# LZ-QWQ/Multi-modal-Tracking

Measured on AMD Instinct MI355X. Metric: tracker FPS (template+search fwd) MixViT-B RGB-T @320px, 1/2/4/8 MI355X, higher is better.
Workload: dtype bf16; 1 GPU; mixformer_vit_rgbt (two-stream) ViT-B 128px template x2 + 320px search, RGB+TIR, 1 frame(s)/GPU/step; variant=rgbt, batch_per_gpu=1, template=128, search=320, hidden=768, depth=12, parallelism=single, hip_graph=True

## Files before the change

multi-modal-tracking_amd/csrc/gemm_glds.hip:

```cpp
#include "common.hpp"
#include "gemm_internal.hpp"

#include <algorithm>

#ifndef MMT_GEMM_ABLATE
#define MMT_GEMM_ABLATE 0
#endif
#ifndef MMT_GEMM_GM
#define MMT_GEMM_GM 8
#endif
#ifndef MMT_GEMM_AB
#define MMT_GEMM_AB 0
#endif
#ifndef MMT_GEMM_OCC2_RES
#define MMT_GEMM_OCC2_RES 1
#endif
#ifndef MMT_GEMM_SK_TICKET_FIRST
#define MMT_GEMM_SK_TICKET_FIRST 0
#endif
#ifndef MMT_GEMM_SK8_MIN
#define MMT_GEMM_SK8_MIN 64
#endif
#ifndef MMT_GEMM_NO_OCC2
#define MMT_GEMM_NO_OCC2 0
#endif

#if MMT_STAMP_BUILD
__device__ unsigned long long g_mmt_stamps[16384 * 8];
extern "C" int mmt_gemm_stamps(unsigned long long* host, int n) {
    return (int)hipMemcpyFromSymbol(host, HIP_SYMBOL(g_mmt_stamps), sizeof(unsigned long long) * n);
}
#endif
#define MMT_STAMP(I, INSN) MMT_STAMP_AT(g_mmt_stamps, I, INSN)

namespace {

template <int N>
struct gemm_ic {
    static constexpr int value = N;
};

typedef __attribute__((address_space(3))) void lds_void;
typedef __attribute__((address_space(1))) void glb_void;

template <int N>
MMT_DEV void wait_vm() {
    asm volatile("s_waitcnt vmcnt(%0)" ::"n"(N) : "memory");
}

MMT_DEV void glds16(const void* src, unsigned char* dst) {
    __builtin_amdgcn_global_load_lds((glb_void*)src, (lds_void*)dst, 16, 0, 0);
}

template <int L, int ST>
MMT_DEV void wait_stages(int ahead) {
    static_assert(ST <= 4, "wait table written for ST <= 4");
    if (ahead <= 0) wait_vm<0>();
    else if (ahead == 1) wait_vm<L>();
    else if (ahead == 2 || ST < 4) wait_vm<(ST >= 3 ? 2 * L : L)>();
    else wait_vm<(ST >= 4 ? 3 * L : L)>();
}

__device__ __attribute__((aligned(64))) const uint32_t g_zero_chunk[16] = {0};
__device__ __attribute__((aligned(64))) const uint32_t g_one_chunk_bf16[4] = {0x3F80u, 0u, 0u, 0u};
__device__ __attribute__((aligned(64))) const uint32_t g_one_chunk_f16[4] = {0x3C00u, 0u, 0u, 0u};

template <int OFF>
MMT_DEV uint2 gemm_tr16(const unsigned char* p) {
    uint2 r;
    const uint32_t a = (uint32_t)(uintptr_t)(const __attribute__((address_space(3))) unsigned char*)p;
    asm volatile("ds_read_b64_tr_b16 %0, %1 offset:%2" : "=v"(r) : "v"(a), "n"(OFF));
    return r;
}

MMT_DEV int gemm_trsw(int k) { return 2 * ((k & 3) | (((k >> 3) & 1) << 2)); }

struct gemm_lean_null {
    MMT_DEV constexpr decltype(nullptr) operator[](int) const { return nullptr; }
};
struct gemm_lean_fixed {
    static constexpr int64_t a_seg_rows = INT32_MAX, a_segs_a = 1, a_stride_a = 0, a_stride_b = 0;
    static constexpr int64_t c_seg_rows = 0, c_seg_pitch = 0;
    static constexpr int32_t k_split = 0, conv_h = 0, conv_up = 1, conv_cin = 0, conv_k3 = 0;
    static constexpr int32_t r_mode = 0, r_p0 = 1, r_p1 = 1, r_t = 0;
    static constexpr float* sk_ws = nullptr;
    static constexpr uint32_t* sk_cnt = nullptr;
    static constexpr int64_t sk_cnt_n = 0;
    gemm_lean_null a1;
};
struct gemm_lean_grid {
    int32_t per_g;
    int32_t tn_magic;
    int32_t q8, r8;
    float inv_k;
};
template <int EPI, int ACT>
struct gemm_lean_args;
template <int ACT>
struct gemm_lean_args<1, ACT> : gemm_lean_fixed, gemm_lean_grid {
    const void *a[2], *w[2];
    const float *bias[2], *ln_colsum[2], *ln_stats_in[2];
    void* c[2];
    int32_t M, N, K, lda, ldc;
    float ln_eps;
    static constexpr int32_t act = ACT, c2_copy = 0, ldr = 0;
    gemm_lean_null r, c2, ln_stats_out;
};
template <int ACT>
struct gemm_lean_args<2, ACT> : gemm_lean_fixed, gemm_lean_grid {
    const void *a[2], *w[2];
    const float *bias[2], *r[2];
    void *c[2], *c2[2];
    float* ln_stats_out[2];
    int32_t M, N, K, lda, ldc, ldr;
    static constexpr int32_t act = 0, c2_copy = 1;
    static constexpr float ln_eps = 0.f;
    gemm_lean_null ln_colsum, ln_stats_in;
};
template <typename P>
struct gemm_is_lean { static constexpr bool value = false; };
template <int EPI, int ACT>
struct gemm_is_lean<gemm_lean_args<EPI, ACT>> { static constexpr bool value = true; };

template <typename T, int BM, int BN, int WGM, int WGN, int KS, int ST, bool CONV, int LNM, int OCC = 1, bool RS = false,
          int EPI = 0, typename P = mmt_gemm_params>
MMT_DEV void gemm_glds_tile(const P& p, const int g, const int tile, const int slice, const int nsk,
                            const int ntiles) {
    constexpr int NW = WGM * WGN, TPG = 64 * NW;
    constexpr int KT = 64;
    constexpr int STAGE = (BM + BN) * 128;
    constexpr int PA = BM / 8 / NW, PB = BN / 8 / NW;
    static_assert(PA * 8 * NW == BM && PB * 8 * NW == BN, "pieces divide evenly over the waves");
    constexpr int L = PA + PB;
    constexpr int WM = BM / WGM, WN = BN / WGN, MT = WM / 16, NT = WN / 16;
    static_assert(KS * ST * STAGE <= 160 * 1024, "LDS budget");
    constexpr bool SB = BM * BN >= 256 * 256 || OCC > 1;
    constexpr bool W4 = BM == 256 && BN == 256 && NW == 4;
    static_assert(!W4 || (KS == 1 && ST == 2 && OCC == 1 && !CONV && (LNM == 0 || LNM == 2)), "impl 9 geometry");
    static_assert(!SB || (KS == 1 && (LNM == 0 || LNM >= 2) && !CONV), "impl 7 / 8 / 9: plain GEMM (or handed-in LN statistics)");
    constexpr bool TA = LNM == 4, TB = LNM == 3 || LNM == 4;
    static_assert(!TB || (BM == 128 && BN == 128 && !CONV), "MN-major operands: 128x128 tiles");
    static_assert(KS == 1 || BM * BN * 4 <= KS * ST * STAGE, "k-group reduction buffer");
    constexpr bool LEAN = gemm_is_lean<P>::value;
    static_assert(!LEAN || (OCC == 1 && !CONV && !RS && (LNM == 0 || LNM == 2) && BM * BN <= 128 * 128 &&
                            ((EPI == 1 && LNM == 2) || (EPI == 2 && LNM == 0))), "lean frame kernels");
    constexpr int LDS_BYTES = W4 ? (BM / 2) * (BN + 4) * 4 + BM * 8 + 64 : KS * ST * STAGE;
    static_assert(LDS_BYTES >= KS * ST * STAGE && LDS_BYTES <= 160 * 1024, "LDS budget");
    __shared__ __attribute__((aligned(1024))) unsigned char lds[LDS_BYTES];
    MMT_STAMP(0, "s_memrealtime");
    MMT_STAMP(1, "s_memtime");

    const int tiles_m = (p.M + BM - 1) / BM;
    constexpr int GM = MMT_GEMM_GM;
    int tm, tn;
    if ((BM * BN >= 256 * 128 || OCC > 1) && gridDim.x * gridDim.y * gridDim.z > 512 && tiles_m > GM) {
        const int tiles_n = ntiles / tiles_m, grp = tile / (GM * tiles_n), first = grp * GM;
        const int gsz = min(tiles_m - first, GM), r = tile - grp * GM * tiles_n;
        tm = first + r % gsz;
        tn = r / gsz;
    } else if constexpr (LEAN) {
        tn = (int)(((uint32_t)tile * (uint32_t)p.tn_magic) >> 16);
        tm = tile - tn * tiles_m;
    } else {
        tm = tile % tiles_m;
        tn = tile / tiles_m;
    }
    constexpr bool LNF = LNM == 1 || LNM == 2;
    const int m0_tile = tm * BM, n0 = tn * BN;
    const int lane = threadIdx.x & 63, kg = threadIdx.x / TPG;
    const int wid = (threadIdx.x % TPG) >> 6, wr = wid / WGN, wc = wid % WGN;
    const int l16 = lane & 15, lg = lane >> 4;
    const int M = p.M, N = p.N, K = p.K;

    const T* A0 = (const T*)p.a[g];
    const T* A1 = (const T*)p.a1[g];
    const T* W = (const T*)p.w[g];

    const int prow = lane >> 3, pch = (lane & 7) ^ prow;
    int64_t aoff[PA], boff[PB];
    int ay[PA], ax[PA];
    const int ch = p.conv_h, cup = CONV ? p.conv_up : 1, hi = CONV ? p.conv_h / cup : 0;
    if constexpr (!CONV) {
        const int segr = (int)p.a_seg_rows, sega = (int)p.a_segs_a;
        const bool plain = segr >= M;
#pragma unroll
        for (int i = 0; i < PA; ++i) {
            const int m = min(m0_tile + (wid * PA + i) * 8 + prow, M - 1);
            if (plain) {
                aoff[i] = (int64_t)m * p.lda;
            } else {
                const int seg = m / segr, sa = seg % sega;
                aoff[i] = sa * p.a_stride_a + (int64_t)((seg - sa) / sega) * p.a_stride_b + (int64_t)(m - seg * segr) * p.lda;
            }
            ay[i] = ax[i] = 0;
        }
    } else {
#pragma unroll
        for (int i = 0; i < PA; ++i) {
            const int m = min(m0_tile + (wid * PA + i) * 8 + prow, M - 1);
            const int b = m / (ch * ch), rem = m - b * ch * ch;
            ay[i] = rem / ch;
// ... 316 lines not shown
#pragma unroll
                for (int nt = 0; nt < NT; ++nt)
#pragma unroll
                    for (int mt = 0; mt < MT; ++mt) acc[nt][mt] += __builtin_bit_cast(f32x4, v[nt][mt]);
            }
        }
    }

    constexpr int TP = BN + 4;
    constexpr int EPASS = BM * TP * 4 + KS * BM * 8 + 16 <= KS * ST * STAGE ? 1 : WGM, EB = BM / EPASS;
    static_assert(EPASS == 1 || (EB == WM && KS == 1 && (LNM == 0 || LNM >= 2)),
                  "multi-pass epilogue: plain GEMM tiles (also with handed-in LayerNorm statistics)");
    static_assert(EB * TP * 4 + KS * BM * 8 + 4 <= LDS_BYTES, "epilogue pass fits in LDS");
    constexpr int FLAG_OFF = EB * TP * 4 + KS * BM * 8;
    float* ctile = (float*)lds;
    float* rstat = ctile + EB * TP;
    constexpr int NTH_E = TPG * KS, TPRW = NTH_E / BM;
    static_assert(TPRW >= 1 && (TPRW & (TPRW - 1)) == 0 && TPRW <= 64, "statistics reduction geometry");
    constexpr int NSP = TPRW >= 2 ? 8 : 16;
    f32x2 stp[NSP];
    const int kp = K / 64, srow = threadIdx.x / TPRW, spart = threadIdx.x % TPRW;
    if constexpr (LNM == 2) {
        const f32x2* st = (const f32x2*)p.ln_stats_in[g] + (int64_t)min(m0_tile + srow, M - 1) * kp;
#pragma unroll
        for (int i = 0; i < NSP; ++i) {
            const int j = spart + i * TPRW;
            stp[i] = j < kp ? st[j] : f32x2{0.f, 0.f};
        }
    }
    constexpr int TPR0 = BN / 8, RPP0 = TPG * KS / TPR0, NPASS0 = EB / RPP0;
    constexpr bool RPRE = EPASS == 1 && NPASS0 <= 8 && BM * BN <= 128 * 128 && OCC == 1;
    const int tc0 = (threadIdx.x % TPR0) * 8, tr0 = threadIdx.x / TPR0, nc0 = min(n0 + tc0, N - 8);
    auto rload = [&](int m, int nc, f32x4& ra, f32x4& rb) {
        const float* R = p.r[g];
        const int64_t csr = p.c_seg_rows > 0 ? p.c_seg_rows : INT64_MAX, csp = p.c_seg_pitch;
        int64_t rr = csr == INT64_MAX ? (int64_t)m : (m / csr) * csp + m % csr;
        if (p.r_mode == 1) rr = m % p.r_p0;
        else if (p.r_mode == 2) {
            const int hw = p.r_p0 * p.r_p0, b = m / hw, rem = m - b * hw;
            const int y = rem / p.r_p0, x = rem - y * p.r_p0, hs = p.r_p0 / p.r_p1;
            rr = (int64_t)b * hs * hs + (int64_t)(y / p.r_p1) * hs + (x / p.r_p1);
        }
        if (p.r_t) {
            const u32x4 u = *(const u32x4*)((const T*)R + rr * p.ldr + nc);
            const f32x2 u0 = unpack2<T>(u[0]), u1 = unpack2<T>(u[1]), u2 = unpack2<T>(u[2]), u3 = unpack2<T>(u[3]);
            ra = f32x4{u0[0], u0[1], u1[0], u1[1]};
            rb = f32x4{u2[0], u2[1], u3[0], u3[1]};
        } else {
            ra = *(const f32x4*)(R + rr * p.ldr + nc);
            rb = *(const f32x4*)(R + rr * p.ldr + nc + 4);
        }
    };
    f32x4 rpa[RPRE ? NPASS0 : 1], rpb[RPRE ? NPASS0 : 1];
    if constexpr (LEAN && EPI == 2) __builtin_assume(p.r[g] != nullptr);
    const bool rpre = RPRE && p.r[g] != nullptr && nsk == 1;
    if constexpr (RPRE) {
        if (rpre) {
#pragma unroll
            for (int i = 0; i < NPASS0; ++i) rload(min(m0_tile + tr0 + i * RPP0, M - 1), nc0, rpa[i], rpb[i]);
        }
    }
    lds_barrier();
    if constexpr (LNM == 2) {
        float sx = 0.f, sxx = 0.f;
#pragma unroll
        for (int i = 0; i < NSP; ++i) {
            sx += stp[i][0];
            sxx += stp[i][1];
        }
#pragma unroll
        for (int o = 1; o < TPRW; o <<= 1) {
            sx += __shfl_xor(sx, o, 64);
            sxx += __shfl_xor(sxx, o, 64);
        }
        if (spart == 0) {
            rstat[srow * 2] = sx;
            rstat[srow * 2 + 1] = sxx;
        }
    }
    if constexpr (LNM == 1) {
#pragma unroll
        for (int j = 0; j < MTW; ++j) {
            const int mt = wc + j * WGN;
            const float sx = lanegroup_sum(lsx[j]), sxx = lanegroup_sum(lsxx[j]);
            if (mt < MT && lg == 0) {
                rstat[(kg * BM + wr * WM + mt * 16 + l16) * 2] = sx;
                rstat[(kg * BM + wr * WM + mt * 16 + l16) * 2 + 1] = sxx;
            }
        }
    }
    if ((KS == 1 || kg == 1) && (EPASS == 1 || wr == 0)) {
#pragma unroll
        for (int nt = 0; nt < NT; ++nt)
#pragma unroll
            for (int mt = 0; mt < MT; ++mt)
                *(f32x4*)(ctile + ((EPASS == 1 ? wr * WM : 0) + mt * 16 + l16) * TP + wc * WN + nt * 16 + lg * 4) =
                    acc[nt][mt];
    }
    if constexpr (KS == 2) {
        lds_barrier();
        if (kg == 0) {
#pragma unroll
            for (int nt = 0; nt < NT; ++nt)
#pragma unroll
                for (int mt = 0; mt < MT; ++mt) {
                    f32x4* t4 = (f32x4*)(ctile + (wr * WM + mt * 16 + l16) * TP + wc * WN + nt * 16 + lg * 4);
                    *t4 = *t4 + acc[nt][mt];
// ... 90 lines not shown
#pragma unroll
        for (int ps = 0; ps < NPASS; ++ps) {
            const int r = tr + ps * RPP, off = slice * SLAB + (r * BN + tc) * 4;
            __builtin_amdgcn_raw_buffer_store_b128(*(const u32x4*)(ctile + r * TP + tc), slabs, off, 0, 16);
            __builtin_amdgcn_raw_buffer_store_b128(*(const u32x4*)(ctile + r * TP + tc + 4), slabs, off + 16, 0, 16);
        }
        asm volatile("s_waitcnt vmcnt(0)" ::: "memory");
        __syncthreads();
        int* flag = (int*)(lds + FLAG_OFF);
        if (threadIdx.x == 0) {
            const uint32_t old = __hip_atomic_fetch_add(p.sk_cnt + tix, 1u, __ATOMIC_RELAXED, __HIP_MEMORY_SCOPE_AGENT);
            const int last = old == (uint32_t)(nsk - 1);
            if (last) __hip_atomic_store(p.sk_cnt + tix, 0u, __ATOMIC_RELAXED, __HIP_MEMORY_SCOPE_AGENT);
            *flag = last;
        }
        __syncthreads();
        if (!*flag) return;
        __builtin_amdgcn_fence(__ATOMIC_ACQUIRE, "wavefront");
#pragma unroll
        for (int ps = 0; ps < NPASS; ++ps) {
            const int r = tr + ps * RPP, off = (r * BN + tc) * 4;
            f32x4 sa = {0.f, 0.f, 0.f, 0.f}, sb = sa;
#pragma unroll
            for (int q0 = 0; q0 < 8; q0 += 4) {
                u32x4 pa[4], pb[4];
#pragma unroll
                for (int j = 0; j < 4; ++j) {
                    const int q = q0 + j;
                    if (q < nsk && q != slice) {
                        pa[j] = __builtin_amdgcn_raw_buffer_load_b128(slabs, q * SLAB + off, 0, 16);
                        pb[j] = __builtin_amdgcn_raw_buffer_load_b128(slabs, q * SLAB + off + 16, 0, 16);
                    }
                }
#pragma unroll
                for (int j = 0; j < 4; ++j) {
                    const int q = q0 + j;
                    if (q < nsk) {
                        if (q == slice) {
                            sa += *(const f32x4*)(ctile + r * TP + tc);
                            sb += *(const f32x4*)(ctile + r * TP + tc + 4);
                        } else {
                            sa += __builtin_bit_cast(f32x4, pa[j]);
                            sb += __builtin_bit_cast(f32x4, pb[j]);
                        }
                    }
                }
            }
            *(f32x4*)(ctile + r * TP + tc) = sa;
            *(f32x4*)(ctile + r * TP + tc + 4) = sb;
        }
    }
#endif
    if constexpr (LEAN) {
        __builtin_assume(bias != nullptr);
        if constexpr (EPI == 2) {
            __builtin_assume(R != nullptr);
            __builtin_assume(C2 != nullptr);
            __builtin_assume(p.ln_stats_out[g] != nullptr);
        }
    }
    const int n = n0 + tc, nc = min(n, N - 8);
    const bool csplit = p.c2_copy == 3 || p.c2_copy == 4;
    float* stats_out = p.c2_copy && !csplit && C2 ? p.ln_stats_out[g] : nullptr;
    const bool colsplit = csplit && n >= N - 8;
    char* Cs = colsplit ? C2 : C;
    if (csplit) C2 = nullptr;
    f32x4 bn0 = {0.f, 0.f, 0.f, 0.f}, bn1 = bn0, cs0 = bn0, cs1 = bn0;
    if (bias) {
        bn0 = *(const f32x4*)(bias + nc);
        bn1 = *(const f32x4*)(bias + nc + 4);
    }
    if constexpr (LNF) {
        cs0 = *(const f32x4*)(p.ln_colsum[g] + nc);
        cs1 = *(const f32x4*)(p.ln_colsum[g] + nc + 4);
    }
    float inv_k;
    if constexpr (LEAN) inv_k = p.inv_k;
    else inv_k = 1.f / (float)K;
    const int64_t csr = p.c_seg_rows > 0 ? p.c_seg_rows : INT64_MAX, csp = p.c_seg_pitch;
    const uint32_t csr32 = (uint32_t)min(csr, (int64_t)INT32_MAX);
    auto crow = [&](int m) -> int64_t {
        if (csr == INT64_MAX) return (int64_t)m;
        const uint32_t qd = (uint32_t)m / csr32;
        return (int64_t)qd * csp + (int64_t)((uint32_t)m - qd * csr32);
    };
    constexpr int PG = NPASS < 4 ? NPASS : 4;
    for (int ep = 0; ep < EPASS; ++ep) {
    if (ep > 0) {
        lds_barrier();
        if (wr == ep) {
#pragma unroll
            for (int nt = 0; nt < NT; ++nt)
#pragma unroll
                for (int mt = 0; mt < MT; ++mt)
                    *(f32x4*)(ctile + (mt * 16 + l16) * TP + wc * WN + nt * 16 + lg * 4) = acc[nt][mt];
        }
        lds_barrier();
    }
    const int m0 = m0_tile + ep * EB;
    if constexpr (EPI == 1) {
        static_assert(!RS, "compact epilogue: no row scale");
#pragma unroll
        for (int i = 0; i < NPASS; ++i) {
            const int r = tr + i * RPP, m = m0 + r;
            f32x4 va = *(const f32x4*)(ctile + r * TP + tc);
            f32x4 vb = *(const f32x4*)(ctile + r * TP + tc + 4);
            if constexpr (LNF) {
                float sx = 0.f, sxx = 0.f;
                constexpr int NQ = LNM == 1 ? KS : 1;
// ... 171 lines not shown
                    *(f32x4*)((float*)Cs + es + 4) = ob;
                    if (C2 && p.c2_copy == 2) {
                        *(u32x4*)((T*)C2 + e) = u32x4{pack2<T>(prea[0], prea[1]), pack2<T>(prea[2], prea[3]),
                                                      pack2<T>(preb[0], preb[1]), pack2<T>(preb[2], preb[3])};
                    } else if (C2 && p.c2_copy) {
                        *(u32x4*)((T*)C2 + e) = u32x4{pack2<T>(sa[0], sa[1]), pack2<T>(sa[2], sa[3]),
                                                      pack2<T>(sb[0], sb[1]), pack2<T>(sb[2], sb[3])};
                    } else if (C2) {
                        *(f32x4*)((float*)C2 + e) = sa;
                        *(f32x4*)((float*)C2 + e + 4) = sb;
                    }
                } else {
                    *(u32x4*)((T*)Cs + es) = u32x4{pack2<T>(oa[0], oa[1]), pack2<T>(oa[2], oa[3]),
                                                 pack2<T>(ob[0], ob[1]), pack2<T>(ob[2], ob[3])};
                    if (C2 && p.c2_copy == 2)
                        *(u32x4*)((T*)C2 + e) = u32x4{pack2<T>(prea[0], prea[1]), pack2<T>(prea[2], prea[3]),
                                                      pack2<T>(preb[0], preb[1]), pack2<T>(preb[2], preb[3])};
                    else if (C2)
                        *(u32x4*)((T*)C2 + e) = u32x4{pack2<T>(sa[0], sa[1]), pack2<T>(sa[2], sa[3]),
                                                      pack2<T>(sb[0], sb[1]), pack2<T>(sb[2], sb[3])};
                }
            }
        }
    }
    }
    }
    MMT_STAMP(5, "s_memtime");
#if MMT_STAMP_BUILD
    asm volatile("s_waitcnt vmcnt(0)" ::: "memory");
#endif
    MMT_STAMP(6, "s_memtime");
    MMT_STAMP(7, "s_memrealtime");
}

MMT_DEV int gemm_xcd_lin() {
    const int nwg = gridDim.x * gridDim.y * gridDim.z;
    const int orig = blockIdx.x + gridDim.x * (blockIdx.y + gridDim.y * blockIdx.z);
    const int xcd = orig & 7, q8 = nwg >> 3, r8 = nwg & 7;
    return (xcd < r8 ? xcd * (q8 + 1) : r8 * (q8 + 1) + (xcd - r8) * q8) + (orig >> 3);
}

template <typename T, int BM, int BN, int WGM, int WGN, int KS, int ST, bool CONV, int LNM, int EPI = 0>
__global__ __launch_bounds__(64 * WGM * WGN * KS)
    __attribute__((amdgpu_waves_per_eu(WGM * WGN * KS / 4, WGM * WGN * KS / 4))) void gemm_glds_kernel(
        const mmt_gemm_params p) {
    const int nsk = gridDim.y;
    const int lin = gemm_xcd_lin();
    const int per_g = gridDim.x * nsk;
    const int g = lin / per_g, rem_t = lin - g * per_g;
    const int tile = rem_t / nsk, slice = rem_t - tile * nsk;
    gemm_glds_tile<T, BM, BN, WGM, WGN, KS, ST, CONV, LNM, 1, false, EPI>(p, g, tile, slice, nsk, gridDim.x);
}

template <typename T, int BM, int BN, int WGM, int WGN, int KS, int ST, int LNM, int EPI, int ACT>
__global__ __launch_bounds__(64 * WGM * WGN * KS)
    __attribute__((amdgpu_waves_per_eu(WGM * WGN * KS / 4, WGM * WGN * KS / 4))) void gemm_glds_frame_kernel(
        const gemm_lean_args<EPI, ACT> p) {
    const int orig = blockIdx.x, xcd = orig & 7;
    const int lin = xcd * p.q8 + min(xcd, p.r8) + (orig >> 3);
    const int g = lin >= p.per_g ? 1 : 0;
    gemm_glds_tile<T, BM, BN, WGM, WGN, KS, ST, false, LNM, 1, false, EPI>(p, g, lin - g * p.per_g, 0, 1, p.per_g);
}

template <typename T, int BM, int BN, int WGM, int WGN, int KS, int ST, bool RS = false, int EPI = 0, int LNM = 0>
__global__ __launch_bounds__(64 * WGM * WGN * KS)
    __attribute__((amdgpu_waves_per_eu(WGM * WGN * KS / 2, WGM * WGN * KS / 2))) void gemm_glds_kernel_occ2(
        const mmt_gemm_params p) {
    const int nsk = gridDim.y;
    const int lin = gemm_xcd_lin();
    const int per_g = gridDim.x * nsk;
    const int g = lin / per_g, rem_t = lin - g * per_g;
    const int tile = rem_t / nsk, slice = rem_t - tile * nsk;
    gemm_glds_tile<T, BM, BN, WGM, WGN, KS, ST, false, LNM, 2, RS, EPI>(p, g, tile, slice, nsk, gridDim.x);
}

template <typename T, int LNM, int EPI = 0>
__global__ __launch_bounds__(512) __attribute__((amdgpu_waves_per_eu(4, 4))) void gemm_glds_kernel_occ2_t(
    const mmt_gemm_params p) {
    const int nsk = gridDim.y;
    const int lin = gemm_xcd_lin();
    const int per_g = gridDim.x * nsk;
    const int g = lin / per_g, rem_t = lin - g * per_g;
    const int tile = rem_t / nsk, slice = rem_t - tile * nsk;
    gemm_glds_tile<T, 128, 128, 2, 4, 1, 2, false, LNM, 2, false, EPI>(p, g, tile, slice, nsk, gridDim.x);
}

#if MMT_GEMM_AB
template <typename T, int LNM, bool RS = false, int EPI = 0>
__global__ __launch_bounds__(256) __attribute__((amdgpu_waves_per_eu(1, 1))) void gemm_glds_kernel_w4(
    const mmt_gemm_params p) {
    const int lin = gemm_xcd_lin();
    const int g = lin / gridDim.x, tile = lin - g * gridDim.x;
    gemm_glds_tile<T, 256, 256, 2, 2, 1, 2, false, LNM, 1, RS, EPI>(p, g, tile, 0, 1, gridDim.x);
}
#endif

constexpr int GEMM_MULTI = 4;
struct gemm_multi_args {
    mmt_gemm_params p[GEMM_MULTI];
    int32_t wg0[GEMM_MULTI + 1];
    int32_t tiles[GEMM_MULTI];
    int32_t n;
};

template <typename T, int BM, int BN, int WGM, int WGN, int KS, int ST, bool CONV>
__global__ __launch_bounds__(64 * WGM * WGN * KS)
    __attribute__((amdgpu_waves_per_eu(WGM * WGN * KS / 4, WGM * WGN * KS / 4))) void gemm_glds_multi_kernel(
        const gemm_multi_args a) {
    const int lin = gemm_xcd_lin();
    int i = 0;
    while (i + 1 < a.n && lin >= a.wg0[i + 1]) ++i;
    const int loc = lin - a.wg0[i], nt = a.tiles[i];
    const int g = loc / nt;
    gemm_glds_tile<T, BM, BN, WGM, WGN, KS, ST, CONV, 0>(a.p[i], g, loc - g * nt, 0, 1, nt);
// ... 56 lines not shown
        if (residual_epilogue(p, true)) hipLaunchKernelGGL((gemm_glds_kernel_w4<T, 0, true, 2>), grid, block, 0, st, p);
        else hipLaunchKernelGGL((gemm_glds_kernel_w4<T, 0, true>), grid, block, 0, st, p);
    } else if (p.ln_fold == 2) {
        if (compact_epilogue(p)) hipLaunchKernelGGL((gemm_glds_kernel_w4<T, 2, false, 1>), grid, block, 0, st, p);
        else hipLaunchKernelGGL((gemm_glds_kernel_w4<T, 2>), grid, block, 0, st, p);
    } else if (compact_epilogue(p)) {
        hipLaunchKernelGGL((gemm_glds_kernel_w4<T, 0, false, 1>), grid, block, 0, st, p);
    } else if (residual_epilogue(p)) {
        hipLaunchKernelGGL((gemm_glds_kernel_w4<T, 0, false, 2>), grid, block, 0, st, p);
    } else {
        hipLaunchKernelGGL((gemm_glds_kernel_w4<T, 0>), grid, block, 0, st, p);
    }
    return 0;
#endif
}

bool aligned(const void* ptr, int bytes) { return ((uintptr_t)ptr & (uintptr_t)(bytes - 1)) == 0; }

bool glds_takes(const mmt_gemm_params& p) {
    if (p.K % 8 || p.N % 8 || p.ldc % 8 || (p.r[0] && p.ldr % 8)) return false;
    if (p.ln_fold && p.conv_h > 0) return false;
    if (p.ln_fold == 2 && (p.a_seg_rows < p.M || p.k_split || p.K % 64 || p.K > 64 * 8 * 2)) return false;
    for (int g = 0; g < p.groups; ++g) {
        if (p.ln_fold == 2 && (!p.ln_stats_in[g] || !aligned(p.ln_stats_in[g], 8))) return false;
        if (p.ln_stats_out[g] && (!p.c2_copy || !p.c2[g] || p.N % 64 || !aligned(p.ln_stats_out[g], 8))) return false;
    }
    if (p.conv_h > 0) {
        const int cup = p.conv_up, hi = p.conv_up > 0 ? p.conv_h / p.conv_up : 0;
        if (cup <= 0 || (cup & (cup - 1)) || hi * cup != p.conv_h) return false;
        const int64_t imgs = (p.M + (int64_t)p.conv_h * p.conv_h - 1) / ((int64_t)p.conv_h * p.conv_h);
        const int64_t pitch = p.a_stride_a > 0 ? p.a_stride_a : (int64_t)hi * hi;
        if ((imgs * pitch * (int64_t)p.lda + p.K) >= ((int64_t)1 << 32) || p.K >= (1 << 24)) return false;
    }
    if (p.lda % 8 || p.a_stride_a % 8 || p.a_stride_b % 8 || p.k_split % 8) return false;
    if (p.a_seg_rows > INT32_MAX || p.a_segs_a > INT32_MAX) return false;
    for (int g = 0; g < p.groups; ++g) {
        if (!aligned(p.c[g], 16) || (p.c2[g] && !aligned(p.c2[g], 16))) return false;
        if (p.bias[g] && !aligned(p.bias[g], 16)) return false;
        if (p.r[g] && !aligned(p.r[g], 16)) return false;
        if (p.ln_fold && (!p.ln_colsum[g] || !aligned(p.ln_colsum[g], 16))) return false;
    }
    return true;
}

struct Cand { int cfg, bm, bn, ks; float fixed_us, step_us; };
constexpr Cand kCands[7] = {{1, 128, 128, 1, 6.0f, 0.52f}, {2, 128, 64, 2, 5.0f, 0.52f}, {3, 64, 64, 2, 3.2f, 0.33f},
                            {4, 128, 128, 1, 6.0f, 0.60f}, {5, 256, 128, 1, 7.0f, 0.70f}, {6, 128, 256, 1, 7.0f, 0.70f},
                            {7, 256, 256, 1, 9.0f, 1.33f}};
int64_t tiles_of(const mmt_gemm_params& p, int bm, int bn) {
    return (int64_t)((p.M + bm - 1) / bm) * ((p.N + bn - 1) / bn);
}


int lean_cfg(const mmt_gemm_params& p) {
    if (p.groups > 2 || p.K % 64 || p.conv_h > 0 || p.k_split || p.a_seg_rows < p.M || p.c_seg_rows || p.a_t || p.w_t ||
        p.row_scale || p.splitk >= 2 || std::max({p.lda, p.ldc, p.ldr}) > INT32_MAX)
        return 0;
    for (int g = 0; g < p.groups; ++g)
        if (!p.bias[g]) return 0;
    int cfg = 0;
    if (p.ln_fold == 2 && p.c2_copy == 0 && p.act <= 1 && compact_epilogue(p)) {
        cfg = 1;
    } else if (p.ln_fold == 0 && residual_epilogue(p)) {
        for (int g = 0; g < p.groups; ++g)
            if (!p.r[g] || !p.c2[g] || !p.ln_stats_out[g]) return 0;
        cfg = 3;
    } else {
        return 0;
    }
    return tiles_of(p, kCands[cfg - 1].bm, kCands[cfg - 1].bn) * p.groups <= 256 ? cfg : 0;
}

template <typename T, int BM, int BN, int WGM, int WGN, int KS, int ST, int LNM, int EPI, int ACT>
void launch_lean(const mmt_gemm_params& p, hipStream_t st) {
    gemm_lean_args<EPI, ACT> a{};
    const int tiles_m = (p.M + BM - 1) / BM, nwg = (int)tiles_of(p, BM, BN) * p.groups;
    a.per_g = nwg / p.groups;
    a.tn_magic = 65536 / tiles_m + 1;
    a.q8 = nwg >> 3;
    a.r8 = nwg & 7;
    a.inv_k = 1.f / (float)p.K;
    for (int g = 0; g < p.groups; ++g) {
        a.a[g] = p.a[g];
        a.w[g] = p.w[g];
        a.bias[g] = p.bias[g];
        a.c[g] = p.c[g];
        if constexpr (EPI == 1) {
            a.ln_colsum[g] = p.ln_colsum[g];
            a.ln_stats_in[g] = p.ln_stats_in[g];
        } else {
            a.r[g] = p.r[g];
            a.c2[g] = p.c2[g];
            a.ln_stats_out[g] = p.ln_stats_out[g];
        }
    }
    a.M = p.M, a.N = p.N, a.K = p.K, a.lda = (int32_t)p.lda, a.ldc = (int32_t)p.ldc;
    if constexpr (EPI == 1) a.ln_eps = p.ln_eps;
    else a.ldr = (int32_t)p.ldr;
    hipLaunchKernelGGL((gemm_glds_frame_kernel<T, BM, BN, WGM, WGN, KS, ST, LNM, EPI, ACT>), dim3(nwg),
                       dim3(64 * WGM * WGN * KS), 0, st, a);
}

}

template <typename T>
int mmt_gemm_glds(const mmt_gemm_params& p, hipStream_t st, int force) {
    if (force < 0 || !glds_takes(p)) return 1;
    const int lcfg = lean_cfg(p);
    const bool no_lean = force == 10;
    if (force == 10) force = lcfg;
    const int nk = (p.K + 63) / 64;
    const Cand* cands = kCands;
    auto max_split = [&](const Cand& c) -> int {
        if (p.ln_fold || !p.sk_ws || !p.sk_cnt) return 1;
        const int64_t t = tiles_of(p, c.bm, c.bn) * p.groups;
        if (2 * t > p.sk_cnt_n) return 1;
        int n = 8;
        while (n > 1 && ((int64_t)n * c.ks > nk || t * n * c.bm * c.bn > p.sk_ws_floats)) --n;
        return n;
    };
    auto cost = [&](const Cand& c, int n) {
        const int64_t wg = tiles_of(p, c.bm, c.bn) * p.groups * n;
        const int steps = (nk + n - 1) / n;
        const float red = n > 1 ? 0.8f + 0.5f * (float)(n - 1) * (float)(c.bm * c.bn) / 16384.f : 0.f;
        return (float)((wg + 255) / 256) * (c.fixed_us + (float)((steps + c.ks - 1) / c.ks) * c.step_us) + red;
    };
    int cfg = force, nsk = 1;
    if (p.row_scale) {
        if (force == 9) return launch_w4<T>(p, st);
        if ((force != 0 && force != 8) || p.ln_fold || p.conv_h > 0 || p.a_t || p.w_t) return 1;
        const dim3 grid((unsigned)tiles_of(p, 128, 128), 1, p.groups);
        if (residual_epilogue(p, true))
            hipLaunchKernelGGL((gemm_glds_kernel_occ2<T, 128, 128, 2, 4, 1, 2, true, 2>), grid, dim3(512), 0, st, p);
        else
            hipLaunchKernelGGL((gemm_glds_kernel_occ2<T, 128, 128, 2, 4, 1, 2, true>), grid, dim3(512), 0, st, p);
        return 0;
    }
    if (p.a_t || p.w_t) {
        if (force != 0 && force != 1 && force != 8) return 1;
        const int64_t t8 = tiles_of(p, 128, 128) * p.groups;
        const bool big = t8 > 256;
        const Cand& c = cands[0];
        if (force == 0 && p.a_t && t8 >= MMT_GEMM_SK8_MIN && p.splitk == 0 && max_split(c) > 1) {
            cfg = 8;
            nsk = (int)std::min<int64_t>(max_split(c), (480 + t8 - 1) / t8);
        } else if (force == 1 || (force == 0 && !big)) {
            cfg = 1;
            const int nmax = p.splitk >= 1 ? std::min(p.splitk, max_split(c)) : max_split(c);
            float best = 1e30f;
            for (int n = (p.splitk >= 2 ? nmax : 1); n <= nmax; ++n) {
                const float t = cost(c, n) * (n > 1 && p.splitk == 0 ? 1.15f : 1.f);
                if (t < best) best = t, nsk = n;
            }
        } else {
            cfg = 8;
            if (p.splitk >= 2) nsk = std::min(p.splitk, max_split(c));
        }
        const int lnm = p.a_t ? 4 : 3;
        const dim3 grid((unsigned)tiles_of(p, 128, 128), nsk, p.groups);
        if (cfg == 8) {
            if (lnm == 4) hipLaunchKernelGGL((gemm_glds_kernel_occ2_t<T, 4>), grid, dim3(512), 0, st, p);
            else if (compact_epilogue(p)) hipLaunchKernelGGL((gemm_glds_kernel_occ2_t<T, 3, 1>), grid, dim3(512), 0, st, p);
            else hipLaunchKernelGGL((gemm_glds_kernel_occ2_t<T, 3>), grid, dim3(512), 0, st, p);
        } else {
            if (lnm == 4) hipLaunchKernelGGL((gemm_glds_kernel<T, 128, 128, 2, 4, 1, 4, false, 4>), grid, dim3(512), 0, st, p);
            else hipLaunchKernelGGL((gemm_glds_kernel<T, 128, 128, 2, 4, 1, 4, false, 3>), grid, dim3(512), 0, st, p);
        }
        return 0;
    }
    if (cfg == 0) {
        float best = 1e30f;
        const bool big = tiles_of(p, 128, 128) * p.groups > 256;
        const bool big7 = big && !p.ln_fold && p.conv_h == 0 && p.act != 1;
        for (int ci = 0; ci < (big7 ? 7 : big ? 6 : 3); ++ci) {
            if (ci == 3 || ci == 4) continue;
            if (ci == 6) {
                const float t = cost(cands[ci], 1);
                if (t < best) best = t, cfg = 7, nsk = 1;
                continue;
            }
            const Cand& c = cands[ci];
            const int nmax = p.splitk >= 1 ? std::min(p.splitk, max_split(c)) : max_split(c);
            for (int n = (p.splitk >= 2 ? nmax : 1); n <= nmax; ++n) {
                const float t = cost(c, n) * (n > 1 && p.splitk == 0 ? 1.15f : 1.f);
                if (t < best) best = t, cfg = c.cfg, nsk = n;
            }
        }
        if (!MMT_GEMM_NO_OCC2 && big && nsk == 1 && p.ln_fold != 1 && p.conv_h == 0 &&
            (MMT_GEMM_OCC2_RES || !p.ln_stats_out[0]) &&
            (cfg == 1 || cfg == 5 || cfg == 6 || cfg == 7 || (p.ln_fold == 2 && (cfg == 2 || cfg == 3))))
            cfg = 8;
    } else if (cfg == 8) {
        nsk = 1;
    } else if (cfg >= 1 && cfg <= 7) {
        const Cand& c = cands[cfg - 1];
        if (no_lean) {
            nsk = 1;
        } else if (p.splitk >= 2) {
            nsk = std::min(p.splitk, max_split(c));
        } else if (p.splitk == 0) {
            float best = 1e30f;
            for (int n = 1; n <= max_split(c); ++n) {
                const float t = cost(c, n) * (n > 1 ? 1.15f : 1.f);
                if (t < best) best = t, nsk = n;
            }
        }
    }
    if (!no_lean && nsk == 1 && cfg != 0 && cfg == lcfg) {
        if (cfg == 3) launch_lean<T, 64, 64, 2, 2, 2, 4, 0, 2, 0>(p, st);
        else if (p.act == 1) launch_lean<T, 128, 128, 2, 4, 1, 4, 2, 1, 1>(p, st);
        else launch_lean<T, 128, 128, 2, 4, 1, 4, 2, 1, 0>(p, st);
        return 0;
    }
    switch (cfg) {
        case 1: launch<T, 128, 128, 2, 4, 1, 4>(p, nsk, st); break;
        case 2: launch<T, 128, 64, 2, 2, 2, 3>(p, nsk, st); break;
        case 3: launch<T, 64, 64, 2, 2, 2, 4>(p, nsk, st); break;
        case 4: launch<T, 128, 128, 2, 2, 1, 4>(p, nsk, st); break;
        case 5: launch<T, 256, 128, 4, 2, 1, 3>(p, nsk, st); break;
        case 6: launch<T, 128, 256, 2, 4, 1, 3>(p, nsk, st); break;
        case 7:
            if (p.ln_fold || p.conv_h > 0 || nsk > 1) return 1;
            hipLaunchKernelGGL((gemm_glds_kernel<T, 256, 256, 4, 2, 1, 2, false, 0>),
                               dim3((unsigned)tiles_of(p, 256, 256), 1, p.groups), dim3(512), 0, st, p);
            break;
        case 8:
            if (p.ln_fold == 1 || p.conv_h > 0 || nsk > 1) return 1;
            {
                const dim3 grid((unsigned)tiles_of(p, 128, 128), nsk, p.groups);
                if (p.ln_fold == 2) {
                    if (compact_epilogue(p))
                        hipLaunchKernelGGL((gemm_glds_kernel_occ2<T, 128, 128, 2, 4, 1, 2, false, 1, 2>), grid, dim3(512), 0, st, p);
                    else
                        hipLaunchKernelGGL((gemm_glds_kernel_occ2<T, 128, 128, 2, 4, 1, 2, false, 0, 2>), grid, dim3(512), 0, st, p);
                } else if (compact_epilogue(p))
                    hipLaunchKernelGGL((gemm_glds_kernel_occ2<T, 128, 128, 2, 4, 1, 2, false, 1>), grid, dim3(512), 0, st, p);
                else if (residual_epilogue(p))
                    hipLaunchKernelGGL((gemm_glds_kernel_occ2<T, 128, 128, 2, 4, 1, 2, false, 2>), grid, dim3(512), 0, st, p);
                else
                    hipLaunchKernelGGL((gemm_glds_kernel_occ2<T, 128, 128, 2, 4, 1, 2>), grid, dim3(512), 0, st, p);
            }
            break;
        case 9: return launch_w4<T>(p, st);
        default: return 1;
    }
    return 0;
}

namespace {
template <typename T, int BM, int BN, int WGM, int WGN, int KS, int ST>
void launch_multi(const mmt_gemm_params* ps, int n, bool conv, hipStream_t st) {
    gemm_multi_args a{};
    a.n = n;
    a.wg0[0] = 0;
    for (int i = 0; i < n; ++i) {
        a.p[i] = ps[i];
        a.tiles[i] = (int32_t)tiles_of(ps[i], BM, BN);
        a.wg0[i + 1] = a.wg0[i] + a.tiles[i] * ps[i].groups;
    }
    const dim3 grid(a.wg0[n]), block(64 * WGM * WGN * KS);
    if (conv) hipLaunchKernelGGL((gemm_glds_multi_kernel<T, BM, BN, WGM, WGN, KS, ST, true>), grid, block, 0, st, a);
    else hipLaunchKernelGGL((gemm_glds_multi_kernel<T, BM, BN, WGM, WGN, KS, ST, false>), grid, block, 0, st, a);
}
}

template <typename T>
int mmt_gemm_glds_multi(const mmt_gemm_params* ps, int n, hipStream_t st) {
    if (n < 1 || n > GEMM_MULTI) return 1;
    const bool conv = ps[0].conv_h > 0;
    const int force = ps[0].impl;
    for (int i = 0; i < n; ++i) {
        const mmt_gemm_params& p = ps[i];
        if (!glds_takes(p) || (p.conv_h > 0) != conv || p.ln_fold || p.impl != force || force < 0 || force > 4 ||
            p.a_t || p.w_t)
            return 1;
    }
    int cfg = force;
    if (cfg == 0) {
        float best = 1e30f;
        for (int ci = 0; ci < 3; ++ci) {
            const Cand& c = kCands[ci];
            int64_t wg = 0;
            float slowest = 0.f;
            for (int i = 0; i < n; ++i) {
                wg += tiles_of(ps[i], c.bm, c.bn) * ps[i].groups;
                const int steps = (ps[i].K + 63) / 64;
                slowest = std::max(slowest, c.fixed_us + (float)((steps + c.ks - 1) / c.ks) * c.step_us);
            }
            const float t = (float)((wg + 255) / 256) * slowest;
            if (t < best) best = t, cfg = c.cfg;
        }
    }
    int64_t wg_total = 0;
    for (int i = 0; i < n; ++i) wg_total += tiles_of(ps[i], kCands[cfg - 1].bm, kCands[cfg - 1].bn) * ps[i].groups;
    if (wg_total > INT32_MAX) return 1;
    switch (cfg) {
        case 1: launch_multi<T, 128, 128, 2, 4, 1, 4>(ps, n, conv, st); break;
        case 2: launch_multi<T, 128, 64, 2, 2, 2, 3>(ps, n, conv, st); break;
        case 3: launch_multi<T, 64, 64, 2, 2, 2, 4>(ps, n, conv, st); break;
        case 4: launch_multi<T, 128, 128, 2, 2, 1, 4>(ps, n, conv, st); break;
        default: return 1;
    }
    return 0;
}

template int mmt_gemm_glds<bf16_t>(const mmt_gemm_params&, hipStream_t, int);
template int mmt_gemm_glds<f16_t>(const mmt_gemm_params&, hipStream_t, int);
template int mmt_gemm_glds_multi<bf16_t>(const mmt_gemm_params*, int, hipStream_t);
template int mmt_gemm_glds_multi<f16_t>(const mmt_gemm_params*, int, hipStream_t);
```

Measured before the change: 1063 frames/s.

## Extend lean frame GEMM kernels to more epilogue forms and paired launches

Widens the lean, compile-time-specialised GEMM path so it also covers plain-bias, GELU, residual-without-LN-stats, two-A-operand k_split and optional-bias fp32 forms, each with a trimmed kernel-argument struct. It also adds a two-problem lean multi kernel that runs a pair of small GEMMs in one launch with XCD-aware workgroup remapping. The goal is to cut per-kernel argument and branch overhead, and the launch count, for the small per-frame GEMMs. In exchange it adds several more template instantiations and more complex dispatch logic.

```diff
diff --git a/multi-modal-tracking_amd/csrc/gemm_glds.hip b/multi-modal-tracking_amd/csrc/gemm_glds.hip
--- a/multi-modal-tracking_amd/csrc/gemm_glds.hip
+++ b/multi-modal-tracking_amd/csrc/gemm_glds.hip
@@ -2,6 +2,7 @@
 #include "gemm_internal.hpp"
 
 #include <algorithm>
+#include <type_traits>
 
 #ifndef MMT_GEMM_ABLATE
 #define MMT_GEMM_ABLATE 0
@@ -81,12 +82,19 @@
 struct gemm_lean_fixed {
     static constexpr int64_t a_seg_rows = INT32_MAX, a_segs_a = 1, a_stride_a = 0, a_stride_b = 0;
     static constexpr int64_t c_seg_rows = 0, c_seg_pitch = 0;
-    static constexpr int32_t k_split = 0, conv_h = 0, conv_up = 1, conv_cin = 0, conv_k3 = 0;
+    static constexpr int32_t conv_h = 0, conv_up = 1, conv_cin = 0, conv_k3 = 0;
     static constexpr int32_t r_mode = 0, r_p0 = 1, r_p1 = 1, r_t = 0;
     static constexpr float* sk_ws = nullptr;
     static constexpr uint32_t* sk_cnt = nullptr;
     static constexpr int64_t sk_cnt_n = 0;
+};
+struct gemm_lean_a_one {
+    static constexpr int32_t k_split = 0;
     gemm_lean_null a1;
+};
+struct gemm_lean_a_two {
+    const void* a1[2];
+    int32_t k_split;
 };
 struct gemm_lean_grid {
     int32_t per_g;
@@ -94,10 +102,11 @@
     int32_t q8, r8;
     float inv_k;
 };
-template <int EPI, int ACT>
+constexpr int LEAN_PLAIN = 1, LEAN_R = 2, LEAN_A2 = 4, LEAN_OPTB = 8;
+template <int EPI, int ACT, int FORM = 0>
 struct gemm_lean_args;
 template <int ACT>
-struct gemm_lean_args<1, ACT> : gemm_lean_fixed, gemm_lean_grid {
+struct gemm_lean_args<1, ACT, 0> : gemm_lean_fixed, gemm_lean_a_one, gemm_lean_grid {
     const void *a[2], *w[2];
     const float *bias[2], *ln_colsum[2], *ln_stats_in[2];
     void* c[2];
@@ -106,8 +115,8 @@
     static constexpr int32_t act = ACT, c2_copy = 0, ldr = 0;
     gemm_lean_null r, c2, ln_stats_out;
 };
-template <int ACT>
-struct gemm_lean_args<2, ACT> : gemm_lean_fixed, gemm_lean_grid {
+template <>
+struct gemm_lean_args<2, 0, 0> : gemm_lean_fixed, gemm_lean_a_one, gemm_lean_grid {
     const void *a[2], *w[2];
     const float *bias[2], *r[2];
     void *c[2], *c2[2];
@@ -117,10 +126,46 @@
     static constexpr float ln_eps = 0.f;
     gemm_lean_null ln_colsum, ln_stats_in;
 };
+template <int ACT>
+struct gemm_lean_args<1, ACT, LEAN_PLAIN> : gemm_lean_fixed, gemm_lean_a_one, gemm_lean_grid {
+    const void *a[2], *w[2];
+    const float* bias[2];
+    void* c[2];
+    int32_t M, N, K, lda, ldc;
+    static constexpr int32_t act = ACT, c2_copy = 0, ldr = 0;
+    static constexpr float ln_eps = 0.f;
+    gemm_lean_null r, c2, ln_stats_out, ln_colsum, ln_stats_in;
+};
+struct gemm_lean_f32_r {
+    const float* r[2];
+    int32_t ldr;
+};
+struct gemm_lean_f32_nor {
+    static constexpr int32_t ldr = 0;
+    gemm_lean_null r;
+};
+template <int FORM>
+struct gemm_lean_args<2, 0, FORM>
+    : gemm_lean_fixed, std::conditional_t<(FORM & LEAN_A2) != 0, gemm_lean_a_two, gemm_lean_a_one>,
+      std::conditional_t<(FORM & LEAN_R) != 0, gemm_lean_f32_r, gemm_lean_f32_nor>, gemm_lean_grid {
+    static_assert(FORM & LEAN_PLAIN, "the hand-off form is FORM 0");
+    const void *a[2], *w[2];
+    const float* bias[2];
+    void* c[2];
+    int32_t M, N, K, lda, ldc;
+    static constexpr int32_t act = 0, c2_copy = 0;
+    static constexpr float ln_eps = 0.f;
+    gemm_lean_null c2, ln_stats_out, ln_colsum, ln_stats_in;
+};
+template <int BYTES>
+MMT_DEV unsigned char* gemm_lds() {
+    __shared__ __attribute__((aligned(1024))) unsigned char lds[BYTES];
+    return lds;
+}
 template <typename P>
-struct gemm_is_lean { static constexpr bool value = false; };
-template <int EPI, int ACT>
-struct gemm_is_lean<gemm_lean_args<EPI, ACT>> { static constexpr bool value = true; };
+struct gemm_is_lean { static constexpr bool value = false; static constexpr int form = 0; };
+template <int EPI, int ACT, int FORM>
+struct gemm_is_lean<gemm_lean_args<EPI, ACT, FORM>> { static constexpr bool value = true; static constexpr int form = FORM; };
 
 template <typename T, int BM, int BN, int WGM, int WGN, int KS, int ST, bool CONV, int LNM, int OCC = 1, bool RS = false,
           int EPI = 0, typename P = mmt_gemm_params>
@@ -142,11 +187,12 @@
     static_assert(!TB || (BM == 128 && BN == 128 && !CONV), "MN-major operands: 128x128 tiles");
     static_assert(KS == 1 || BM * BN * 4 <= KS * ST * STAGE, "k-group reduction buffer");
     constexpr bool LEAN = gemm_is_lean<P>::value;
-    static_assert(!LEAN || (OCC == 1 && !CONV && !RS && (LNM == 0 || LNM == 2) && BM * BN <= 128 * 128 &&
-                            ((EPI == 1 && LNM == 2) || (EPI == 2 && LNM == 0))), "lean frame kernels");
+    constexpr int LFORM = gemm_is_lean<P>::form;
+    static_assert(!LEAN || (OCC == 1 && !CONV && !RS && BM * BN <= 128 * 128 &&
+                            ((EPI == 1 && LNM == (LFORM ? 0 : 2)) || (EPI == 2 && LNM == 0))), "lean frame kernels");
     constexpr int LDS_BYTES = W4 ? (BM / 2) * (BN + 4) * 4 + BM * 8 + 64 : KS * ST * STAGE;
     static_assert(LDS_BYTES >= KS * ST * STAGE && LDS_BYTES <= 160 * 1024, "LDS budget");
-    __shared__ __attribute__((aligned(1024))) unsigned char lds[LDS_BYTES];
+    unsigned char* const lds = gemm_lds<LDS_BYTES>();
     MMT_STAMP(0, "s_memrealtime");
     MMT_STAMP(1, "s_memtime");
 
@@ -569,7 +615,8 @@
         }
     };
     f32x4 rpa[RPRE ? NPASS0 : 1], rpb[RPRE ? NPASS0 : 1];
-    if constexpr (LEAN && EPI == 2) __builtin_assume(p.r[g] != nullptr);
+    constexpr bool LEAN_HAS_R = LEAN && EPI == 2 && (LFORM == 0 || (LFORM & LEAN_R));
+    if constexpr (LEAN_HAS_R) __builtin_assume(p.r[g] != nullptr);
     const bool rpre = RPRE && p.r[g] != nullptr && nsk == 1;
     if constexpr (RPRE) {
         if (rpre) {
@@ -766,9 +813,9 @@
     }
 #endif
     if constexpr (LEAN) {
-        __builtin_assume(bias != nullptr);
-        if constexpr (EPI == 2) {
-            __builtin_assume(R != nullptr);
+        if constexpr (!(LFORM & LEAN_OPTB)) __builtin_assume(bias != nullptr);
+        if constexpr (LEAN_HAS_R) __builtin_assume(R != nullptr);
+        if constexpr (EPI == 2 && LFORM == 0) {
             __builtin_assume(C2 != nullptr);
             __builtin_assume(p.ln_stats_out[g] != nullptr);
         }
@@ -1046,14 +1093,38 @@
     gemm_glds_tile<T, BM, BN, WGM, WGN, KS, ST, CONV, LNM, 1, false, EPI>(p, g, tile, slice, nsk, gridDim.x);
 }
 
-template <typename T, int BM, int BN, int WGM, int WGN, int KS, int ST, int LNM, int EPI, int ACT>
+template <typename T, int BM, int BN, int WGM, int WGN, int KS, int ST, int LNM, int EPI, int ACT, int FORM = 0>
 __global__ __launch_bounds__(64 * WGM * WGN * KS)
     __attribute__((amdgpu_waves_per_eu(WGM * WGN * KS / 4, WGM * WGN * KS / 4))) void gemm_glds_frame_kernel(
-        const gemm_lean_args<EPI, ACT> p) {
+        const gemm_lean_args<EPI, ACT, FORM> p) {
     const int orig = blockIdx.x, xcd = orig & 7;
     const int lin = xcd * p.q8 + min(xcd, p.r8) + (orig >> 3);
     const int g = lin >= p.per_g ? 1 : 0;
     gemm_glds_tile<T, BM, BN, WGM, WGN, KS, ST, false, LNM, 1, false, EPI>(p, g, lin - g * p.per_g, 0, 1, p.per_g);
+}
+
+template <typename P0, typename P1>
+struct gemm_lean_multi_args {
+    P0 p0;
+    P1 p1;
+    int32_t wg1;
+    int32_t q8, r8;
+};
+template <typename T, int BM, int BN, int WGM, int WGN, int KS, int ST, int EPI0, typename P0, int EPI1, typename P1>
+__global__ __launch_bounds__(64 * WGM * WGN * KS)
+    __attribute__((amdgpu_waves_per_eu(WGM * WGN * KS / 4, WGM * WGN * KS / 4))) void gemm_glds_frame_multi_kernel(
+        const gemm_lean_multi_args<P0, P1> a) {
+    const int orig = blockIdx.x, xcd = orig & 7;
+    const int lin = xcd * a.q8 + min(xcd, a.r8) + (orig >> 3);
+    if (lin < a.wg1) {
+        const int g = lin >= a.p0.per_g ? 1 : 0;
+        gemm_glds_tile<T, BM, BN, WGM, WGN, KS, ST, false, 0, 1, false, EPI0>(a.p0, g, lin - g * a.p0.per_g, 0, 1,
+                                                                             a.p0.per_g);
+    } else {
+        const int loc = lin - a.wg1, g = loc >= a.p1.per_g ? 1 : 0;
+        gemm_glds_tile<T, BM, BN, WGM, WGN, KS, ST, false, 0, 1, false, EPI1>(a.p1, g, loc - g * a.p1.per_g, 0, 1,
+                                                                             a.p1.per_g);
+    }
 }
 
 template <typename T, int BM, int BN, int WGM, int WGN, int KS, int ST, bool RS = false, int EPI = 0, int LNM = 0>
@@ -1216,52 +1287,84 @@
 }
 
 
-int lean_cfg(const mmt_gemm_params& p) {
-    if (p.groups > 2 || p.K % 64 || p.conv_h > 0 || p.k_split || p.a_seg_rows < p.M || p.c_seg_rows || p.a_t || p.w_t ||
+int lean_cfg(const mmt_gemm_params& p, int* form = nullptr, bool opt_bias = false) {
+    if (p.groups > 2 || p.K % 64 || p.conv_h > 0 || p.a_seg_rows < p.M || p.c_seg_rows || p.a_t || p.w_t ||
         p.row_scale || p.splitk >= 2 || std::max({p.lda, p.ldc, p.ldr}) > INT32_MAX)
         return 0;
+    bool has_bias = p.bias[0] != nullptr, has_r = p.r[0] != nullptr;
     for (int g = 0; g < p.groups; ++g)
-        if (!p.bias[g]) return 0;
-    int cfg = 0;
-    if (p.ln_fold == 2 && p.c2_copy == 0 && p.act <= 1 && compact_epilogue(p)) {
+        if ((p.bias[g] != nullptr) != has_bias || (p.r[g] != nullptr) != has_r) return 0;
+    int cfg = 0, f = 0;
+    if (p.k_split) {
+        if (p.k_split % 64 || p.k_split >= p.K || p.ln_fold || !residual_epilogue(p) || p.c2[0] || p.c2[p.groups - 1])
+            return 0;
+        cfg = 3, f = LEAN_PLAIN | LEAN_A2 | (has_r ? LEAN_R : 0);
+    } else if (p.ln_fold == 2 && p.c2_copy == 0 && p.act <= 1 && compact_epilogue(p)) {
         cfg = 1;
     } else if (p.ln_fold == 0 && residual_epilogue(p)) {
-        for (int g = 0; g < p.groups; ++g)
-            if (!p.r[g] || !p.c2[g] || !p.ln_stats_out[g]) return 0;
-        cfg = 3;
+        bool any = false, all = true;
+        for (int g = 0; g < p.groups; ++g) {
+            const bool h = p.c2[g] && p.ln_stats_out[g];
+            if (!h && (p.c2[g] || p.ln_stats_out[g])) return 0;
+            any |= h, all &= h;
+        }
+        if (any != all || (all && !has_r)) return 0;
+        cfg = 3, f = all ? 0 : LEAN_PLAIN | (has_r ? LEAN_R : 0);
+    } else if (p.ln_fold == 0 && p.c2_copy == 0 && (p.act == 0 || p.act == 2) && compact_epilogue(p)) {
+        cfg = p.act == 2 ? 2 : 3, f = LEAN_PLAIN;
     } else {
         return 0;
     }
+    if (!has_bias) {
+        if (!(opt_bias && (f & LEAN_PLAIN) && p.c_f32)) return 0;
+        f |= LEAN_OPTB;
+    }
+    if (form) *form = f;
     return tiles_of(p, kCands[cfg - 1].bm, kCands[cfg - 1].bn) * p.groups <= 256 ? cfg : 0;
 }
 
-template <typename T, int BM, int BN, int WGM, int WGN, int KS, int ST, int LNM, int EPI, int ACT>
-void launch_lean(const mmt_gemm_params& p, hipStream_t st) {
-    gemm_lean_args<EPI, ACT> a{};
-    const int tiles_m = (p.M + BM - 1) / BM, nwg = (int)tiles_of(p, BM, BN) * p.groups;
-    a.per_g = nwg / p.groups;
+mmt_gemm_params lean_view(const mmt_gemm_params& p) {
+    mmt_gemm_params v = p;
+    if (v.r_mode == 1 && v.r_p0 >= v.M) v.r_mode = 0;
+    return v;
+}
+
+template <int BM, int BN, int EPI, int ACT, int FORM>
+void fill_lean(gemm_lean_args<EPI, ACT, FORM>& a, const mmt_gemm_params& p, int nwg_all) {
+    const int tiles_m = (p.M + BM - 1) / BM;
+    a.per_g = (int)tiles_of(p, BM, BN);
     a.tn_magic = 65536 / tiles_m + 1;
-    a.q8 = nwg >> 3;
-    a.r8 = nwg & 7;
+    a.q8 = nwg_all >> 3;
+    a.r8 = nwg_all & 7;
     a.inv_k = 1.f / (float)p.K;
     for (int g = 0; g < p.groups; ++g) {
         a.a[g] = p.a[g];
         a.w[g] = p.w[g];
         a.bias[g] = p.bias[g];
         a.c[g] = p.c[g];
-        if constexpr (EPI == 1) {
+        if constexpr (EPI == 1 && FORM == 0) {
             a.ln_colsum[g] = p.ln_colsum[g];
             a.ln_stats_in[g] = p.ln_stats_in[g];
-        } else {
-            a.r[g] = p.r[g];
+        }
+        if constexpr (EPI == 2 && FORM == 0) {
             a.c2[g] = p.c2[g];
             a.ln_stats_out[g] = p.ln_stats_out[g];
         }
+        if constexpr (EPI == 2 && (FORM == 0 || (FORM & LEAN_R))) a.r[g] = p.r[g];
+        if constexpr ((FORM & LEAN_A2) != 0) a.a1[g] = p.a1[g];
     }
     a.M = p.M, a.N = p.N, a.K = p.K, a.lda = (int32_t)p.lda, a.ldc = (int32_t)p.ldc;
-    if constexpr (EPI == 1) a.ln_eps = p.ln_eps;
-    else a.ldr = (int32_t)p.ldr;
-    hipLaunchKernelGGL((gemm_glds_frame_kernel<T, BM, BN, WGM, WGN, KS, ST, LNM, EPI, ACT>), dim3(nwg),
+    if constexpr (EPI == 1 && FORM == 0) a.ln_eps = p.ln_eps;
+    if constexpr (EPI == 2 && (FORM == 0 || (FORM & LEAN_R))) a.ldr = (int32_t)p.ldr;
+    if constexpr ((FORM & LEAN_A2) != 0) a.k_split = p.k_split;
+}
+
+template <typename T, int BM, int BN, int WGM, int WGN, int KS, int ST, int LNM, int EPI, int ACT, int FORM = 0>
+void launch_lean(const mmt_gemm_params& p, hipStream_t st) {
+    gemm_lean_args<EPI, ACT, FORM> a{};
+    const int nwg = (int)tiles_of(p, BM, BN) * p.groups;
+    fill_lean<BM, BN>(a, p, nwg);
+    hipLaunchKernelGGL((gemm_glds_frame_kernel<T, BM, BN, WGM, WGN, KS, ST, LNM, EPI, ACT, FORM>), dim3(nwg),
                        dim3(64 * WGM * WGN * KS), 0, st, a);
 }
 
@@ -1270,7 +1373,9 @@
 template <typename T>
 int mmt_gemm_glds(const mmt_gemm_params& p, hipStream_t st, int force) {
     if (force < 0 || !glds_takes(p)) return 1;
-    const int lcfg = lean_cfg(p);
+    const mmt_gemm_params pv = lean_view(p);
+    int lform = 0;
+    const int lcfg = lean_cfg(pv, &lform);
     const bool no_lean = force == 10;
     if (force == 10) force = lcfg;
     const int nk = (p.K + 63) / 64;
@@ -1371,9 +1476,16 @@
         }
     }
     if (!no_lean && nsk == 1 && cfg != 0 && cfg == lcfg) {
-        if (cfg == 3) launch_lean<T, 64, 64, 2, 2, 2, 4, 0, 2, 0>(p, st);
-        else if (p.act == 1) launch_lean<T, 128, 128, 2, 4, 1, 4, 2, 1, 1>(p, st);
-        else launch_lean<T, 128, 128, 2, 4, 1, 4, 2, 1, 0>(p, st);
+        constexpr int PL = LEAN_PLAIN, PR = LEAN_PLAIN | LEAN_R, A2 = LEAN_A2;
+        if (cfg == 1 && p.act == 1) launch_lean<T, 128, 128, 2, 4, 1, 4, 2, 1, 1>(pv, st);
+        else if (cfg == 1) launch_lean<T, 128, 128, 2, 4, 1, 4, 2, 1, 0>(pv, st);
+        else if (cfg == 2) launch_lean<T, 128, 64, 2, 2, 2, 3, 0, 1, 2, PL>(pv, st);
+        else if (lform == 0) launch_lean<T, 64, 64, 2, 2, 2, 4, 0, 2, 0>(pv, st);
+        else if (!p.c_f32) launch_lean<T, 64, 64, 2, 2, 2, 4, 0, 1, 0, PL>(pv, st);
+        else if (lform == PL) launch_lean<T, 64, 64, 2, 2, 2, 4, 0, 2, 0, PL>(pv, st);
+        else if (lform == PR) launch_lean<T, 64, 64, 2, 2, 2, 4, 0, 2, 0, PR>(pv, st);
+        else if (lform == (PL | A2)) launch_lean<T, 64, 64, 2, 2, 2, 4, 0, 2, 0, PL | A2>(pv, st);
+        else launch_lean<T, 64, 64, 2, 2, 2, 4, 0, 2, 0, PR | A2>(pv, st);
         return 0;
     }
     switch (cfg) {
@@ -1426,16 +1538,40 @@
     if (conv) hipLaunchKernelGGL((gemm_glds_multi_kernel<T, BM, BN, WGM, WGN, KS, ST, true>), grid, block, 0, st, a);
     else hipLaunchKernelGGL((gemm_glds_multi_kernel<T, BM, BN, WGM, WGN, KS, ST, false>), grid, block, 0, st, a);
 }
+
+template <typename T>
+bool launch_lean_multi(const mmt_gemm_params* ps, int n, hipStream_t st) {
+    constexpr int BM = 64, BN = 64, F1 = LEAN_PLAIN | LEAN_R | LEAN_A2 | LEAN_OPTB;
+    using P0 = gemm_lean_args<1, 0, LEAN_PLAIN>;
+    using P1 = gemm_lean_args<2, 0, F1>;
+    if (n != 2) return false;
+    const mmt_gemm_params v0 = lean_view(ps[0]), v1 = lean_view(ps[1]);
+    int f0 = 0, f1 = 0;
+    if (lean_cfg(v0, &f0, true) != 3 || lean_cfg(v1, &f1, true) != 3) return false;
+    if (v0.c_f32 || f0 != LEAN_PLAIN || (f1 | LEAN_OPTB) != F1) return false;
+    const int wg0 = (int)tiles_of(v0, BM, BN) * v0.groups, wg1 = (int)tiles_of(v1, BM, BN) * v1.groups;
+    if (wg0 + wg1 > 256) return false;
+    gemm_lean_multi_args<P0, P1> a{};
+    fill_lean<BM, BN>(a.p0, v0, wg0 + wg1);
+    fill_lean<BM, BN>(a.p1, v1, wg0 + wg1);
+    a.wg1 = wg0;
+    a.q8 = (wg0 + wg1) >> 3;
+    a.r8 = (wg0 + wg1) & 7;
+    hipLaunchKernelGGL((gemm_glds_frame_multi_kernel<T, BM, BN, 2, 2, 2, 4, 1, P0, 2, P1>), dim3(wg0 + wg1), dim3(512),
+                       0, st, a);
+    return true;
+}
 }
 
 template <typename T>
 int mmt_gemm_glds_multi(const mmt_gemm_params* ps, int n, hipStream_t st) {
     if (n < 1 || n > GEMM_MULTI) return 1;
     const bool conv = ps[0].conv_h > 0;
-    const int force = ps[0].impl;
+    const bool no_lean = ps[0].impl == 10;
+    const int force = no_lean ? 0 : ps[0].impl;
     for (int i = 0; i < n; ++i) {
         const mmt_gemm_params& p = ps[i];
-        if (!glds_takes(p) || (p.conv_h > 0) != conv || p.ln_fold || p.impl != force || force < 0 || force > 4 ||
+        if (!glds_takes(p) || (p.conv_h > 0) != conv || p.ln_fold || p.impl != ps[0].impl || force < 0 || force > 4 ||
             p.a_t || p.w_t)
             return 1;
     }
@@ -1458,6 +1594,7 @@
     int64_t wg_total = 0;
     for (int i = 0; i < n; ++i) wg_total += tiles_of(ps[i], kCands[cfg - 1].bm, kCands[cfg - 1].bn) * ps[i].groups;
     if (wg_total > INT32_MAX) return 1;
+    if (cfg == 3 && !conv && !no_lean && launch_lean_multi<T>(ps, n, st)) return 0;
     switch (cfg) {
         case 1: launch_multi<T, 128, 128, 2, 4, 1, 4>(ps, n, conv, st); break;
         case 2: launch_multi<T, 128, 64, 2, 2, 2, 3>(ps, n, conv, st); break;
```

New measurement: 1085 frames/s (median of 6 runs). 1.02x the previous value.
